# riddhiman13/predictive-multi-agent-framework

Measured on AMD Instinct MI355X. Metric: agent_rollouts_per_s, higher is better.
Workload: dtype f64; 1 GPU; C2: 64 agents x 200-step horizon, 32 sphere obstacles + repulsive sentinel, 1 population(s) per GPU (1 in the job) on 1 GPU(s), static obstacles, one pmaf_tick per step; agents=64, horizon=200, obstacles=32, populations_per_gpu=1, populations_total=1, parallelism=population-per-gpu x1 (same scene on every GPU), devices_visible=1, lanes_per_agent=64, rollout_blocks=64

## Files before the change

### include/pmaf.h

```cpp
#ifndef PMAF_H
#define PMAF_H

#include <stddef.h>
#include <stdint.h>

#ifdef __cplusplus
extern "C" {
#endif

#define PMAF_ABI_VERSION 7

typedef enum pmaf_status {
  PMAF_OK = 0,
  PMAF_ERR_INVALID = -1,
  PMAF_ERR_DEVICE = -2,
  PMAF_ERR_STATE = -3,
  PMAF_ERR_NOMEM = -4
} pmaf_status;

typedef enum pmaf_agent_type {
  PMAF_REAL_AGENT = 0,
  PMAF_GOAL_HEURISTIC = 1,
  PMAF_OBSTACLE_HEURISTIC = 2,
  PMAF_GOAL_OBSTACLE_HEURISTIC = 3,
// ... 141 lines not shown
int pmaf_set_profiling(pmaf_planner *h, int32_t enable);
int pmaf_get_launch_count(pmaf_planner *h, int64_t *launches);
int pmaf_get_kernel_stats(pmaf_planner *h, double *rollout_ms, int64_t *launches,
                          int64_t *agent_steps);
int pmaf_reset_kernel_stats(pmaf_planner *h);
int pmaf_get_launch_config(pmaf_planner *h, int32_t *lanes_per_agent,
                           int32_t *n_blocks, int32_t *lds_bytes);
int pmaf_get_waves_per_agent(pmaf_planner *h, int32_t *waves_per_agent, int32_t *obstacles_per_wave);
int pmaf_get_priority_slices(pmaf_planner *h, int32_t *enabled, int32_t *slice_ticks, int32_t *younger_of_8);
int32_t pmaf_pick_lanes_per_agent(int32_t n_agents, int32_t n_populations, int32_t n_field_obstacles, int32_t n_simds);
double pmaf_estimate_rollout_us(int32_t lanes_per_agent, int32_t n_agents, int32_t n_populations, int32_t n_field_obstacles,
                                int32_t horizon, int32_t n_simds);

int pmaf_debug_external_rollout(pmaf_planner *h, const char *code_object_path, const char *kernel_name);
int pmaf_debug_withhold_mailbox(pmaf_planner *h, int32_t enable);

int pmaf_debug_math(int32_t op, int32_t n, const double *a, const double *b, double *out);

#ifdef __cplusplus
}
#endif
#endif
```

### predictive-multi-agent-framework_amd/csrc/pmaf_host.cpp

```cpp
#include <hip/hip_runtime_api.h>
#include <unistd.h>

#include <cmath>
#include <cstdio>
#include <cstdlib>
#include <cstring>
#include <string>
#include <algorithm>
#include <chrono>
#include <thread>
#include <vector>

#include "../../include/pmaf.h"
#include "pmaf_comm.hpp"
#include "pmaf_types.hpp"
#include "pmaf_lpa_model.hpp"

#ifndef PMAF_W64_SLICE_DEFAULT
#define PMAF_W64_SLICE_DEFAULT true
#endif

using namespace pmaf;

static thread_local std::string g_err;
// ... 39 lines not shown
  size_t lds_rollout = 0, lds_manager = 0;
  hipModule_t ext_mod = nullptr;
  hipFunction_t ext_fn = nullptr;
  hipStream_t stream = nullptr;
  hipEvent_t ev_mgr = nullptr;
  uint64_t mailbox_seq = 0;
  double tick_timeout_s = 5.0;
  bool dbg_withhold = false;
  double *h_wp = nullptr, *d_wp = nullptr, *h_wph = nullptr, *d_wph = nullptr;
  std::vector<int32_t> wp_np, wp_agent;
  double wp_seq = 0.0;
  std::chrono::steady_clock::time_point last_tick_entry{};
  bool wp_timed = true;
  std::vector<double> wp_us;
  bool closest_dirty = true;
  std::vector<double> last_live;
  std::vector<double> live_resident;
  void note_live_obstacles(const double *obstacles) {
    const size_t row = (size_t)D.n_obs * 7, field = (size_t)(D.n_obs - 1) * 7;
    bool same = last_live.size() == (size_t)D.P * field;
    for (int p = 0; p < D.P && same; p++)
      same = std::memcmp(last_live.data() + p * field, obstacles + p * row, sizeof(double) * field) == 0;
    if (same) return;
    last_live.resize((size_t)D.P * field);
    for (int p = 0; p < D.P; p++) std::memcpy(last_live.data() + p * field, obstacles + p * row, sizeof(double) * field);
    closest_dirty = true;
  }
  bool uses_closest_table() const {
    const int M = D.n_obs - 1;
    const int tiles64 = (M >= 61 && M <= 64) ? 2 : (M + 63) / 64;
    return lpa == 64 && tiles64 >= 2 && tiles64 <= 4 && !force_generic;
  }
  static constexpr size_t TICK_RING = 8192;
  std::vector<float> tick_enq_us, tick_sp_us;
  size_t tick_head = 0, tick_count = 0;
  std::vector<void *> allocs;
  std::vector<size_t> alloc_bytes;
  double *h_out = nullptr;
  std::vector<double> real_pos_h, real_vel_h, real_force_h;
  double *d_out = nullptr;
  double *h_zc = nullptr, *d_zc = nullptr;
// ... 261 lines not shown

static void ensure_scores(pmaf_planner *h) {
  if (h->scores_valid) return;
  pmaf_k_launch_score(h->D, h->cp, h->stream);
  HIP_CHECK(hipGetLastError());
  h->scores_valid = true;
}

static const double *stage_live_obstacles_zero_copy(pmaf_planner *h, const double *obstacles) {
  if (!obstacles) return nullptr;
  const size_t n = (size_t)h->D.P * h->D.n_obs * 7;
  if (!h->peer.on && h->live_resident.size() == n && std::memcmp(h->live_resident.data(), obstacles, sizeof(double) * n) == 0) return nullptr;
  check_range(obstacles, n, "obstacles");
  h->note_live_obstacles(obstacles);
  h->live_resident.assign(obstacles, obstacles + n);
  aos_to_soa(obstacles, h->h_zc, h->D.P, h->D.n_obs);
  return h->d_zc;
}

struct ResidentGuard {
  pmaf_planner *h; bool armed = true;
  ~ResidentGuard() { if (armed) { h->live_resident.clear(); h->last_live.clear(); h->closest_dirty = true; } }
};

static void flush_real_position(pmaf_planner *h) {
  if (!h->real_pos_pending) return;
  sync(h);
  h->upload(h->D.real_pos, h->real_pos_h.data(), (size_t)h->D.P * 3);
  h->real_pos_pending = false;
}

static void launch_manager(pmaf_planner *h, const ManagerArgs &A0, hipEvent_t done = nullptr) {
  ManagerArgs A = A0;
  const bool hand_over_position = h->real_pos_pending;
  if (hand_over_position) {
    if (h->D.P <= PMAF_RP_INLINE) {
      A.real_pos_inline = 1;
      std::memcpy(A.real_pos_val, h->h_rp, sizeof(double) * 3 * (size_t)h->D.P);
    } else {
      A.real_pos_src = h->d_rp;
    }
  }
  if (A.do_reset) h->paths_gen++;
  if (A.do_reset && h->uses_closest_table()) { A.compute_closest = h->closest_dirty ? 1 : 0; h->closest_dirty = false; }
  A.tuned_real_step = (h->math == MATH_XACT && !h->force_generic) ? 1 : 0;
  pmaf_k_launch_manager(h->D, h->cp, A, h->lds_manager, h->stream, done);
  HIP_CHECK(hipGetLastError());
  if (hand_over_position) h->real_pos_pending = false;
}

static void refresh_real_cache(pmaf_planner *h) {
  for (int p = 0; p < h->D.P; p++) {
    const double *o = h->h_out + p * PMAF_MBOX;
    for (int c = 0; c < 3; c++) {
      h->real_pos_h[p * 3 + c] = o[1 + c];
      h->real_vel_h[p * 3 + c] = o[4 + c];
      h->real_force_h[p * 3 + c] = o[8 + c];
    }
  }
}

static void wait_mailbox(pmaf_planner *h, double seq, const char *who = "pmaf_tick") {
// ... 316 lines not shown
    REQUIRE(h->lds_manager <= 160 * 1024,
            "pmaf_create: n_agents + obstacle table exceed the manager kernel's LDS budget (160 KB: 8 B per agent, 60 B per obstacle)");
    HIP_CHECK(pmaf_k_set_lds_limits(h->lds_manager, h->lds_rollout));

    size_t PN = (size_t)P * N;
    double *goal = h->dalloc<double>(P * 3);
    D.goal = goal;
    D.agent_init_pos = h->dalloc<double>(P * 3);
    D.start_pos = h->dalloc<double>(P * 3);
    D.start_vel = h->dalloc<double>(P * 3);
    D.obs_start = h->dalloc<double>((size_t)P * 7 * n_obs);
    D.known_start = h->dalloc<int32_t>((size_t)P * n_obs);
    D.obs_live = h->dalloc<double>((size_t)P * 7 * n_obs);
    D.closest_idx = h->dalloc<int32_t>((size_t)P * n_obs);
    D.closest_ok = h->dalloc<int32_t>((size_t)P);
    double *ka = h->dalloc<double>(PN), *kc = h->dalloc<double>(PN), *kr = h->dalloc<double>(PN), *kd = h->dalloc<double>(PN);
    D.k_attr = ka; D.k_circ = kc; D.k_repel = kr; D.k_damp = kd;
    int32_t *types = h->dalloc<int32_t>(N);
    D.types = types;
    D.rot = h->dalloc<double>(PN * 3 * n_obs);
    double *rnd = h->dalloc<double>(PN * 3 * n_obs);
    D.rnd = rnd;
    D.paths = h->dalloc<double>(PN * (size_t)cap * 3);
    D.n_points = h->dalloc<int32_t>(PN);
    D.agent_vel = h->dalloc<double>(PN * 3);
    D.min_obs = h->dalloc<double>(PN);
    D.cost_ws = h->dalloc<double>(PN);
    D.path_len = h->dalloc<double>(PN);
    D.goal_dist = h->dalloc<double>(PN);
    D.reached = h->dalloc<int32_t>(PN);
// ... 81 lines not shown
        int p = (int)(pa / N);
        for (int c = 0; c < 3; c++) paths[pa * cap * 3 + c] = init[p * 3 + c];
        av[pa * 3] = 0.01;
      }
      h->upload(D.paths, paths.data(), paths.size());
      h->upload(D.n_points, np.data(), np.size());
      h->upload(D.min_obs, mo.data(), mo.size());
      h->upload(D.agent_vel, av.data(), av.size());
    }
    h->real_pos_h = init;
    h->real_vel_h = v0;
    h->real_force_h.assign(P * 3, 0.0);
    h->real_path.assign(P, {});
    for (int p = 0; p < P; p++) h->real_path[p].insert(h->real_path[p].end(), {init[p * 3], init[p * 3 + 1], init[p * 3 + 2]});
    h->rollout_pending = true;
    sync(h);
    *out = h;
  });
  if (rc != PMAF_OK && h) { pmaf_destroy(h); }
  return rc;
}

int pmaf_destroy(pmaf_planner *h) {
  if (!h) return PMAF_OK;
  (void)hipSetDevice(h->device);
  if (h->stream) (void)hipStreamSynchronize(h->stream);
  detach_comm(h);
  peer_disconnect(h);
  if (h->d_send1) (void)hipFree(h->d_send1);
  if (h->ext_mod) (void)hipModuleUnload(h->ext_mod);
// ... 17 lines not shown
}

int pmaf_set_initial_position(pmaf_planner *h, const double *pos) {
  return guarded([&] {
    REQUIRE(h && pos, "pmaf_set_initial_position: NULL argument");
    check_range(pos, (size_t)h->D.P * 3, "pmaf_set_initial_position");
    h->use_device();
    sync(h);
    DevView &D = h->D;
    const int P = D.P;
    h->upload(D.agent_init_pos, pos, P * 3);
    h->upload(D.real_init_pos, pos, P * 3);
    h->upload(D.real_pos, pos, P * 3);
    h->real_pos_pending = false;
    h->upload(D.start_pos, pos, P * 3);
    h->paths_gen++;
    pmaf_k_launch_restart_paths(D, D.start_pos, h->stream);
    HIP_CHECK(hipGetLastError());
    h->real_pos_h.assign(pos, pos + P * 3);
    for (int p = 0; p < P; p++)
      h->real_path[p].insert(h->real_path[p].end(), {pos[p * 3], pos[p * 3 + 1], pos[p * 3 + 2]});
    sync(h);
    h->scores_valid = false;
    h->rollout_pending = true;
    h->stepped = false;
  });
}

int pmaf_set_real_position(pmaf_planner *h, const double *pos) {
  return guarded([&] {
// ... 288 lines not shown
  const int P = h->D.P;
  check_range(pos, (size_t)P * 3, "pos");
  if (vel) check_range(vel, (size_t)P * 3, "vel");
  h->use_device();
  sync(h);
  std::vector<double> in((size_t)P * 6, 0.0);
  for (int p = 0; p < P; p++)
    for (int c = 0; c < 3; c++) { in[p * 6 + c] = pos[p * 3 + c]; if (vel) in[p * 6 + 3 + c] = vel[p * 3 + c]; }
  std::vector<double> pk((size_t)P * 6);
  for (int p = 0; p < P; p++)
    for (int c = 0; c < 3; c++) { pk[p * 3 + c] = in[p * 6 + c]; pk[(size_t)P * 3 + p * 3 + c] = in[p * 6 + 3 + c]; }
  h->upload(h->d_reset_in, pk.data(), pk.size());
  h->paths_gen++;
  pmaf_k_launch_set_agents(h->D, h->d_reset_in, vel ? h->d_reset_in + (size_t)P * 3 : nullptr, h->stream);
  HIP_CHECK(hipGetLastError());
  sync(h);
  h->scores_valid = false;
  h->rollout_pending = false;
  h->stepped = true;
}

int pmaf_set_agent_positions(pmaf_planner *h, const double *pos) {
  return guarded([&] {
    REQUIRE(h && pos, "pmaf_set_agent_positions: NULL argument");
    set_agents(h, pos, nullptr);
  });
}

int pmaf_set_agent_pos_and_vels(pmaf_planner *h, const double *pos, const double *vel) {
  return guarded([&] {
// ... 549 lines not shown

int pmaf_get_health(pmaf_planner *h, int32_t *bits) {
  return guarded([&] {
    REQUIRE(h && bits, "pmaf_get_health: NULL argument");
    for (int p = 0; p < h->D.P; p++) bits[p] = (int32_t)h->h_out[p * PMAF_MBOX + 15];
  });
}

int pmaf_debug_withhold_mailbox(pmaf_planner *h, int32_t enable) {
  return guarded([&] {
    REQUIRE(h, "pmaf_debug_withhold_mailbox: NULL handle");
    h->dbg_withhold = enable != 0;
  });
}

int pmaf_enable_winner_path(pmaf_planner *h, int32_t enable) {
  return guarded([&] {
    REQUIRE(h, "pmaf_enable_winner_path: NULL handle");
    h->use_device();
    sync(h);
    if (!enable) {
      if (h->h_wp) { (void)hipHostFree(h->h_wp); h->h_wp = nullptr; h->d_wp = nullptr; }
      if (h->h_wph) { (void)hipHostFree(h->h_wph); h->h_wph = nullptr; h->d_wph = nullptr; }
      h->wp_seq = 0.0;
      return;
    }
    if (h->h_wp) return;
    const size_t P = (size_t)h->D.P;
    HIP_CHECK(hipHostMalloc((void **)&h->h_wp, sizeof(double) * P * h->D.cap * 3, hipHostMallocMapped));
    HIP_CHECK(hipHostGetDevicePointer((void **)&h->d_wp, h->h_wp, 0));
// ... 159 lines not shown
      uint64_t n = 0;
      REQUIRE(r + sizeof(n) <= end, "pmaf_load_state: blob truncated");
      std::memcpy(&n, r, sizeof(n)); r += sizeof(n);
      REQUIRE(r + sizeof(double) * n <= end, "pmaf_load_state: blob truncated");
      rp.assign(reinterpret_cast<const double *>(r), reinterpret_cast<const double *>(r) + n);
      r += sizeof(double) * n;
    }
    h->paths_gen++;
    h->cp_valid = hd.cp_valid != 0;
    h->scores_valid = hd.scores_valid != 0;
    h->rollout_pending = hd.rollout_pending != 0;
    h->stepped = hd.stepped != 0;
    h->real_pos_pending = false;
    h->has_best_h = -1;
    h->closest_dirty = true;
    h->last_live.clear();
    h->live_resident.clear();
  });
}

void *pmaf_stream(pmaf_planner *h) { return h ? (void *)h->stream : nullptr; }

int pmaf_set_profiling(pmaf_planner *h, int32_t enable) {
  return guarded([&] {
    REQUIRE(h, "pmaf_set_profiling: NULL handle");
    h->use_device();
    sync(h);
    h->profiling = enable != 0;
    h->prof_every = enable > 1 ? enable : 1;
    h->prof_phase = 0;
// ... 102 lines not shown
```

### predictive-multi-agent-framework_amd/csrc/pmaf_k_misc.hip

```cpp
#include <mutex>
#include <hip/hip_runtime.h>
#include <hip/hip_ext.h>

#include "pmaf_types.hpp"
#include "pmaf_device.hpp"
#include "pmaf_rollout_w64.hpp"
#include "pmaf_rollout_grp.hpp"

using namespace pmaf;

template <int LPA>
__global__ __launch_bounds__(64) void k_rollout(DevView D, CostParams CP) {
  extern __shared__ double smem[];
  const int lane = threadIdx.x;
  const int pop = blockIdx.y;
  constexpr int APW = 64 / LPA;
  const int sub = lane % LPA;
  const int grp = lane / LPA;
  const int a = blockIdx.x * APW + grp;
  const bool active = a < D.N;
  const int aa = active ? a : 0;
  const int n_obs = D.n_obs;
  const PopConst C = D.C;
  const unsigned long long t_begin = wall_clock64();
// ... 209 lines not shown
  int best = D.best_idx[pop];
  const int had_best = D.has_best[pop];
  const int old_best_id = D.best_id[pop];
  int htype = D.best_type[pop];
  const double *rp_src = A.real_pos_src ? A.real_pos_src : D.real_pos;
  V3 rp;
  if (A.real_pos_inline) rp = mk(A.real_pos_val[pop * 3], A.real_pos_val[pop * 3 + 1], A.real_pos_val[pop * 3 + 2]);
  else rp = mk(rp_src[pop * 3], rp_src[pop * 3 + 1], rp_src[pop * 3 + 2]);
  if ((A.real_pos_src || A.real_pos_inline) && !A.do_move && lane == 0) {
    D.real_pos[pop * 3] = rp.x; D.real_pos[pop * 3 + 1] = rp.y; D.real_pos[pop * 3 + 2] = rp.z;
  }
  V3 rv = mk(D.real_vel[pop * 3], D.real_vel[pop * 3 + 1], D.real_vel[pop * 3 + 2]);
  V3 rf = mk(D.real_force[pop * 3], D.real_force[pop * 3 + 1], D.real_force[pop * 3 + 2]);
  const V3 init_pos = mk(D.real_init_pos[pop * 3], D.real_init_pos[pop * 3 + 1], D.real_init_pos[pop * 3 + 2]);
  int32_t *rk = D.real_known + (size_t)pop * n_obs;
  double *live_dev = D.obs_live + (size_t)pop * 7 * n_obs;
  const double *live = A.live_src ? A.live_src + (size_t)pop * 7 * n_obs : live_dev;
  if (A.do_move || A.do_reset) {
    if (A.live_src) {
      const int total = 7 * n_obs;
      for (int base = 0; base < total; base += 64 * 8) {
        double v[8];
#pragma unroll
        for (int k = 0; k < 8; k++) {
          const int i = base + k * 64 + lane;
          v[k] = (i < total) ? __builtin_nontemporal_load(live + i) : 0.0;
        }
#pragma unroll
        for (int k = 0; k < 8; k++) {
          const int i = base + k * 64 + lane;
          if (i < total) { smem[i] = v[k]; live_dev[i] = v[k]; }
        }
      }
    } else {
      for (int i = lane; i < 7 * n_obs; i += 64) smem[i] = live[i];
    }
    for (int i = lane; i < n_obs; i += 64) s_known[i] = rk[i];
  }
  unsigned long long peer_wait = 0ull;
  int peer_status = 0;
  const PeerView *PV = A.peer;
  const bool peer_on = PV != nullptr && A.do_select && A.do_move && A.do_reset;
  if (peer_on) {
    const int src_rank = PV->couple[pop * 2], src_pop = PV->couple[pop * 2 + 1];
    if (src_rank >= 0) {
      const double want = A.peer_tick - 1.0;
      const double *slot = PV->inbox + ((((size_t)((long long)want & 1) * PV->world + src_rank) * PV->P + src_pop) * PMAF_PEER_SLOT);
      const unsigned long long t0 = wall_clock64();
      for (;;) {
        const double got = __hip_atomic_load(slot + 8, __ATOMIC_ACQUIRE, __HIP_MEMORY_SCOPE_SYSTEM);
        if (got == want) break;
        if (got > want) { peer_status = 2; break; }
// ... 75 lines not shown
      const double *src = D.rnd + ((size_t)pop * N + min_idx) * 3 * n_obs;
      double *dst = D.best_rnd + (size_t)pop * 3 * n_obs;
      for (int i = lane; i < 3 * n_obs; i += 64) dst[i] = src[i];
      rand_g = src;
      htype = D.types[min_idx];
      if (lane == 0) {
        D.has_best[pop] = 1;
        D.best_id[pop] = min_idx + 1;
        D.best_type[pop] = htype;
      }
    }
    best = min_idx;
    if (lane == 0) D.best_idx[pop] = best;
  }
  PMAF_MSEC();
  if (A.do_move) {
    int gid = A.agent_id_inline ? A.agent_id_val[pop] : (A.agent_id ? A.agent_id[pop] : best);
    size_t pg = (size_t)pop * N + gid;
    double k_attr = D.k_attr[pg], k_circ = D.k_circ[pg], k_repel = D.k_repel[pg], k_damp = D.k_damp[pg];
    wave_lds_fence();
    const int ntiles = (M + 63) / 64;
    unsigned long long kb = 0ull;
    V3 F = mk(0.0, 0.0, 0.0);
    bool acc_clamped = false;
    if (A.tuned_real_step && ntiles <= 4) {
      double *rrot = D.real_rot + (size_t)pop * 3 * n_obs;
      double *clist = s_cost + N + (N & 1);
      unsigned kb32 = 0u;
      if (ntiles <= 1)
        real_step_w64<1>(D, A.dt_real, pop, lane, htype, smem, s_known, rrot, rand_g, clist, k_attr, k_circ, k_repel,
// ... 15 lines not shown
      bool gate = !(dg < C.approach || (norm(rv) < 0.5 * C.vel_max && norm(rp - init_pos) < 0.2));
      double scale = 1.0, dummy_min = C.shell;
      circ_and_scale<64, true>(gate, lane, 0, htype, rp, rv, goal, g, C, k_circ, T, n_obs,
                               D.real_rot + (size_t)pop * 3 * n_obs, rand_g, kb, dummy_min, F, scale);
      V3 new_pos;
      finish_step(rp, rv, g, F, scale, C, k_attr, k_repel, k_damp, A.dt_real, T.pos(n_obs - 1), T.r[n_obs - 1], new_pos);
      rp = new_pos;
      acc_clamped = norm((C.mass != 1.0) ? (F / C.mass) : F) > 13.0;
    }
    if (acc_clamped) health |= PMAF_HB_ACC_CLAMPED;
    rf = F;
    for (int t = 0; t < ntiles; t++) {
      int i = t * 64 + lane;
      if (i < M) {
        const int32_t f = (int32_t)((kb >> t) & 1ull);
        rk[i] = f;
        s_known[i] = f;
      }
    }
    if (lane == 0) {
      D.real_pos[pop * 3] = rp.x; D.real_pos[pop * 3 + 1] = rp.y; D.real_pos[pop * 3 + 2] = rp.z;
      D.real_vel[pop * 3] = rv.x; D.real_vel[pop * 3 + 1] = rv.y; D.real_vel[pop * 3 + 2] = rv.z;
      D.real_force[pop * 3] = F.x; D.real_force[pop * 3 + 1] = F.y; D.real_force[pop * 3 + 2] = F.z;
    }
  }

  PMAF_MSEC();
  double hv[PMAF_WINNER_HDR];
  const bool want_hdr = A.do_select && (A.winner_hdr != nullptr || peer_on);
  if (want_hdr) {
    const size_t pb = (size_t)pop * N + best;
    hv[0] = s_cost[best];
    hv[1] = (double)best;
    hv[2] = (double)D.n_points[pb];
// ... 62 lines not shown
    double *wh = A.wp_hdr + pop * 4;
    if (lane == 0) { wh[0] = (double)(n3 / 3); wh[1] = (double)best; wh[2] = 0.0; }
    __threadfence_system();
    if (lane == 0) *reinterpret_cast<volatile double *>(wh + 3) = A.seq;
  }
  if (A.do_reset) {
    V3 sp, sv;
    if (A.reset_from_real) { sp = rp; sv = rv; }
    else if (A.reset_in_inline) {
      sp = mk(A.reset_in_val[pop * 6], A.reset_in_val[pop * 6 + 1], A.reset_in_val[pop * 6 + 2]);
      sv = mk(A.reset_in_val[pop * 6 + 3], A.reset_in_val[pop * 6 + 4], A.reset_in_val[pop * 6 + 5]);
    } else { sp = reset_sp; sv = reset_sv; }
    double vn = norm(sv);
    if (vn > C.vel_max) sv = (C.vel_max / vn) * sv;
    wave_lds_fence();
    double *st = D.obs_start + (size_t)pop * 7 * n_obs;
    for (int i = lane; i < 6 * n_obs; i += 64) st[i] = smem[i];
    int32_t *ks = D.known_start + (size_t)pop * n_obs;
    for (int i = lane; i < n_obs; i += 64) ks[i] = s_known[i];
    if (!A.rollout_follows) {
      for (int a = lane; a < N; a += 64) {
        size_t pa = (size_t)pop * N + a;
        double *path = D.paths + pa * (size_t)D.cap * 3;
        path[0] = sp.x; path[1] = sp.y; path[2] = sp.z;
        D.n_points[pa] = 1;
        D.agent_vel[pa * 3] = sv.x; D.agent_vel[pa * 3 + 1] = sv.y; D.agent_vel[pa * 3 + 2] = sv.z;
        D.min_obs[pa] = C.shell;
      }
      int32_t *ko = D.known_out + (size_t)pop * N * n_obs;
      for (int k = lane; k < N * n_obs; k += 64) ko[k] = s_known[k % n_obs];
    }
    if (lane == 0) {
      D.start_pos[pop * 3] = sp.x; D.start_pos[pop * 3 + 1] = sp.y; D.start_pos[pop * 3 + 2] = sp.z;
      D.start_vel[pop * 3] = sv.x; D.start_vel[pop * 3 + 1] = sv.y; D.start_vel[pop * 3 + 2] = sv.z;
    }
    if (A.compute_closest) {
      bool mv = false;
      for (int i = lane; i < M; i += 64) {
        const V3 ov = T.vel(i);
        mv = mv || !(ov.x == 0.0 && ov.y == 0.0 && ov.z == 0.0);
      }
      mv = wave_any(mv);
      if (!mv) {
        int32_t *ci = D.closest_idx + (size_t)pop * n_obs;
        for (int i = lane; i < M; i += 64) ci[i] = closest_other(T, n_obs, i, T.pos(i));
      }
      if (lane == 0) D.closest_ok[pop] = mv ? 0 : 1;
    }
  }
// ... 180 lines not shown
  const int pop = idx / D.N;
  const V3 q = mk(pos[pop * 3], pos[pop * 3 + 1], pos[pop * 3 + 2]);
  double *path = D.paths + (size_t)idx * D.cap * 3;
  path[0] = q.x; path[1] = q.y; path[2] = q.z;
  D.n_points[idx] = 1;
  V3 w = mk(0.0, 0.0, 0.0);
  if (vel) {
    w = mk(vel[pop * 3], vel[pop * 3 + 1], vel[pop * 3 + 2]);
    const double vn = norm(w);
    if (vn > D.C.vel_max) w = (D.C.vel_max / vn) * w;
    D.agent_vel[idx * 3] = w.x; D.agent_vel[idx * 3 + 1] = w.y; D.agent_vel[idx * 3 + 2] = w.z;
  }
  if (idx % D.N == 0) {
    D.start_pos[pop * 3] = q.x; D.start_pos[pop * 3 + 1] = q.y; D.start_pos[pop * 3 + 2] = q.z;
    if (vel) { D.start_vel[pop * 3] = w.x; D.start_vel[pop * 3 + 1] = w.y; D.start_vel[pop * 3 + 2] = w.z; }
  }
}

__global__ void k_eval_obstacle_distance(DevView D, const double *obs, double *out) {
  const int idx = blockIdx.x * blockDim.x + threadIdx.x;
  if (idx >= D.P * D.N) return;
  const int pop = idx / D.N;
  const int n_obs = D.n_obs;
  const double *o = obs + (size_t)pop * 7 * n_obs;
  const double *path = D.paths + (size_t)idx * D.cap * 3;
  const int n = D.n_points[idx];
  const V3 p = mk(path[(n - 1) * 3], path[(n - 1) * 3 + 1], path[(n - 1) * 3 + 2]);
  double min_dist = D.C.shell;
  for (int k = 0; k < n_obs; k++) {
    const double d = norm(p - mk(o[k], o[n_obs + k], o[2 * n_obs + k])) - (D.C.rad + o[6 * n_obs + k]);
// ... 126 lines not shown
```

### predictive-multi-agent-framework_amd/csrc/pmaf_k_w64.hip

```cpp
#include <hip/hip_runtime.h>
#include <hip/hip_ext.h>

#include "pmaf_types.hpp"
#include "pmaf_device.hpp"
#include "pmaf_rollout_w64.hpp"
#include "pmaf_rollout_grp.hpp"

using namespace pmaf;

__device__ __forceinline__ double *w64_exp_lds() {
  __shared__ double s_expk[EXPK_N];
  return s_expk;
}
template <int TILES>
__device__ __forceinline__ auto w64_exp_consts(int lane) {
  if constexpr (TILES >= 2) {
    double *tab = w64_exp_lds();
    exp_consts_to_lds(tab, lane);
    wave_lds_fence();
    return exp_consts_from_lds(tab);
  } else {
    return exp_consts_in_vgprs();
  }
}
// ... 252 lines not shown
    D.cost_ws[pa] = cost_ws;
    D.path_len[pa] = path_len;
    D.goal_dist[pa] = dg;
    if (ran) D.reached[pa] = dg < 0.100001;
    atomicAdd(D.step_counter, (unsigned long long)(n - 1));
    D.pred_ticks[pa] = wall_clock64() - t_begin;
  }
}

template <int TILES, int MATH, bool DPPSUM, bool PLAIN, bool SLICE>
__device__ __forceinline__ void rollout_w64_dispatch(const DevView &D, const CostParams &CP) {
  const int lane = threadIdx.x;
  const int pop = blockIdx.y;
  const int a = blockIdx.x;
  if (TILES == 1) {
    const int n_obs = D.n_obs, M = n_obs - 1;
    const double *src = D.obs_start + (size_t)pop * 7 * n_obs;
    const V3 sp = mk(src[M], src[n_obs + M], src[2 * n_obs + M]);
    const V3 sv = mk(src[3 * n_obs + M], src[4 * n_obs + M], src[5 * n_obs + M]);
    const V3 p0 = mk(D.start_pos[pop * 3], D.start_pos[pop * 3 + 1], D.start_pos[pop * 3 + 2]);
    const PopConst C0 = D.C;
    const bool reach = sentinel_reachable(p0, sp, sv, D.zsent_lt[pop], C0, D.cap);
    bool rest = true;
    for (int i = lane; i < M; i += 64) {
      const unsigned long long bx = (unsigned long long)__double_as_longlong(src[3 * n_obs + i]),
                               by = (unsigned long long)__double_as_longlong(src[4 * n_obs + i]),
                               bz = (unsigned long long)__double_as_longlong(src[5 * n_obs + i]);
      rest = rest && ((bx | by | bz) == 0ull);
    }
    const bool st = !wave_any(!rest) && (M <= 59 || !reach);
#define PMAF_BODY(T) \
    if (st) { \
      if (!reach) rollout_w64_body<TILES, T, MATH, 0, DPPSUM, PLAIN, true, SLICE>(D, CP, lane, pop, a); \
      else rollout_w64_body<TILES, T, MATH, 1, DPPSUM, PLAIN, true, SLICE>(D, CP, lane, pop, a); \
    } else if (!reach) rollout_w64_body<TILES, T, MATH, 0, DPPSUM, PLAIN, false, SLICE>(D, CP, lane, pop, a); \
    else rollout_w64_body<TILES, T, MATH, 1, DPPSUM, PLAIN, false, SLICE>(D, CP, lane, pop, a)
    switch (D.types[a]) {
      case T_GOAL: PMAF_BODY(T_GOAL); break;
      case T_OBST: PMAF_BODY(T_OBST); break;
      case T_GOALOBST: PMAF_BODY(T_GOALOBST); break;
      case T_VEL: PMAF_BODY(T_VEL); break;
      case T_RANDOM: PMAF_BODY(T_RANDOM); break;
      case T_HAD: PMAF_BODY(T_HAD); break;
      default: break;
    }
#undef PMAF_BODY
    return;
  }
  switch (D.types[a]) {
    case T_GOAL: rollout_w64_body<TILES, T_GOAL, MATH, 2, DPPSUM, PLAIN>(D, CP, lane, pop, a); break;
    case T_OBST: rollout_w64_body<TILES, T_OBST, MATH, 2, DPPSUM, PLAIN>(D, CP, lane, pop, a); break;
    case T_GOALOBST: rollout_w64_body<TILES, T_GOALOBST, MATH, 2, DPPSUM, PLAIN>(D, CP, lane, pop, a); break;
// ... 55 lines not shown
```

### predictive-multi-agent-framework_amd/csrc/pmaf_types.hpp

```cpp
#pragma once
#include <hip/hip_runtime_api.h>
#include <stddef.h>
#include <stdint.h>

#define PMAF_WINNER_HDR 8
#define PMAF_MBOX 16
#define PMAF_HB_SETPOINT_NAN 1
#define PMAF_HB_FORCE_NAN 2
#define PMAF_HB_ACC_CLAMPED 4
#define PMAF_HB_COST_NAN 8
#define PMAF_PEER_SLOT 16
#define PMAF_PEER_MAX_WORLD 64

namespace pmaf {

enum : int { MATH_IEEE = 0, MATH_FAST = 1, MATH_XACT = 2, MATH_FMA = 3 };

constexpr int pmaf_list_area_doubles(int slots_per_lane) { return (64 * (slots_per_lane <= 2 ? 2 : 4) + 8 + 64) * 4; }

struct PopConst {
  double dt, vel_max, approach, shell, mass, rad;
  double zf_gt, zacc_gt, zinit_lt, zvhalf_lt, zv09_lt;
};

// ... 25 lines not shown
  double *costs;
  double *real_pos, *real_vel, *real_force, *real_init_pos;
  int32_t *real_known;
  double *real_rot;
  int32_t *has_best, *best_id, *best_type;
  double *best_rnd;
  int32_t *best_idx;
  unsigned long long *step_counter;
  unsigned long long *pred_ticks;
  const double *zsent_lt;
  int ablate;
  int n_simds;
  int prio_slice_log2, prio_younger_of_8;
  int32_t *closest_idx;
  int32_t *closest_ok;
};

struct CostParams {
  double k_goal_dist, k_path_len, k_safe_dist, k_workspace;
  double ws[6];
};


struct PeerView {
  int world, rank, P, pad;
  double *inbox;
  double *peer[PMAF_PEER_MAX_WORLD];
  const int32_t *couple;
  const double *couple_radius;
  unsigned long long timeout_ticks;
// ... 2 lines not shown
struct ManagerArgs {
  int do_select, do_move, do_reset;
  int reset_from_real;
  int rollout_follows;
  int tuned_real_step;
  const double *live_src;
  double dt_real;
  const int32_t *agent_id;
  const double *reset_in;
  double *out;
  double seq;
  const PeerView *peer;
  double peer_tick;
  double *winner_hdr;
  int winner_stride;
  int compute_closest;
  double *wp_out;
  double *wp_hdr;
  const double *real_pos_src;
  int real_pos_inline;
  double real_pos_val[3 * 4];
  int agent_id_inline;
  int32_t agent_id_val[4];
  int reset_in_inline;
  double reset_in_val[6 * 4];
};
#define PMAF_RP_INLINE 4

struct PlanArgs {
  const double *obs;
// ... 30 lines not shown
```

### predictive-multi-agent-framework_amd/planner.py

```python
import ctypes as C
import os

import numpy as np

_HERE = os.path.dirname(os.path.abspath(__file__))
VARIANT = os.environ.get("PMAF_VARIANT", "")
LIB_PATH = os.environ.get("PMAF_LIB_PATH") or os.path.join(_HERE, "lib_" + VARIANT if VARIANT else "lib", "libpmaf_hip.so")

_dp = C.POINTER(C.c_double)
_ip = C.POINTER(C.c_int32)


class PmafError(RuntimeError):
    def __init__(self, code, msg):
        super().__init__("pmaf status %d: %s" % (code, msg))
        self.code = code


class PmafParams(C.Structure):
    _fields_ = [
        ("abi_version", C.c_int32), ("n_populations", C.c_int32), ("n_agents", C.c_int32),
        ("n_obstacles", C.c_int32), ("max_prediction_steps", C.c_int32), ("device", C.c_int32),
        ("lanes_per_agent", C.c_int32), ("flags", C.c_int32),
        ("dt", C.c_double), ("velocity_max", C.c_double), ("approach_dist", C.c_double),
# ... 72 lines not shown
    "pmaf_get_kernel_stats": (C.c_int, [_V, _dp, C.POINTER(C.c_int64), C.POINTER(C.c_int64)]),
    "pmaf_reset_kernel_stats": (C.c_int, [_V]),
    "pmaf_get_launch_count": (C.c_int, [_V, C.POINTER(C.c_int64)]),
    "pmaf_get_launch_config": (C.c_int, [_V, _ip, _ip, _ip]),
    "pmaf_get_waves_per_agent": (C.c_int, [_V, _ip, _ip]),
    "pmaf_get_priority_slices": (C.c_int, [_V, _ip, _ip, _ip]),
    "pmaf_pick_lanes_per_agent": (C.c_int32, [C.c_int32, C.c_int32, C.c_int32, C.c_int32]),
    "pmaf_estimate_rollout_us": (C.c_double, [C.c_int32, C.c_int32, C.c_int32, C.c_int32, C.c_int32, C.c_int32]),
    "pmaf_debug_math": (C.c_int, [C.c_int32, C.c_int32, _dp, _dp, _dp]),
    "pmaf_debug_external_rollout": (C.c_int, [_V, C.c_char_p, C.c_char_p]),
    "pmaf_get_health": (C.c_int, [_V, _ip]),
    "pmaf_enable_winner_path": (C.c_int, [_V, C.c_int32]),
    "pmaf_view_winner_path": (C.c_int, [_V, C.POINTER(_dp), C.POINTER(_ip), C.POINTER(_ip)]),
    "pmaf_get_winner_path_times_us": (C.c_int, [_V, _dp, C.c_int32, _ip]),
    "pmaf_debug_withhold_mailbox": (C.c_int, [_V, C.c_int32]),
    "pmaf_peer_info": (C.c_int, [_V, _ip, _ip]),
}


def debug_math(op, a, b=None):
    L = load_library()
    a = np.ascontiguousarray(a, dtype=np.float64)
    b = np.ascontiguousarray(a if b is None else b, dtype=np.float64)
    out = np.zeros_like(a)
    rc = L.pmaf_debug_math(op, a.size, a.ctypes.data_as(_dp), b.ctypes.data_as(_dp), out.ctypes.data_as(_dp))
    if rc != 0:
        raise PmafError(rc, L.pmaf_last_error().decode())
    return out

_LIB = None
# ... 316 lines not shown
        paths = [full[p, :n[p]].copy() for p in range(self.P)]
        return (paths[0], int(n[0]), int(a[0])) if self.P == 1 else (paths, n, a)

    def winner_path_wait(self):
        self._chk(self.L.pmaf_view_winner_path(self._h, None, None, None))

    def winner_path_times_us(self, max_n=1 << 16):
        out = np.zeros(max_n)
        n = C.c_int32(0)
        self._chk(self.L.pmaf_get_winner_path_times_us(self._h, _p(out), max_n, C.byref(n)))
        return out[:n.value].copy()

    def debug_withhold_mailbox(self, enable=True):
        self._chk(self.L.pmaf_debug_withhold_mailbox(self._h, 1 if enable else 0))

    def peer_info(self):
        f, w = C.c_int32(0), C.c_int32(0)
        self._chk(self.L.pmaf_peer_info(self._h, C.byref(f), C.byref(w)))
        return {"fine_grained": bool(f.value), "world": w.value}

    PEER_HANDLE_BYTES = 128

    def peer_export(self, world):
        buf = (C.c_ubyte * self.PEER_HANDLE_BYTES)()
        self._chk(self.L.pmaf_peer_export(self._h, int(world), C.cast(buf, C.c_void_p)))
        return bytes(buf)

    def peer_connect(self, world, rank, handles):
        blob = b"".join(handles)
        assert len(blob) == world * self.PEER_HANDLE_BYTES
# ... 171 lines not shown
```

Before: 270,000 rollouts/s.

## Precompute rollout dispatch facts in manager and skip redundant start-state copies

The manager kernel now computes, once per reset, whether all obstacles are at rest and whether the sentinel is reachable, and stores both in a small device array. Each rollout block reads these flags instead of rescanning the obstacle velocities and re-running the reachability test. The manager also skips rewriting obs_start and known_start when host-side flags show they are already in sync, and it batches the LDS fill of the obstacle and known arrays. In exchange it adds invalidation bookkeeping across reset, set-position and peer paths, with a risk of using stale flags if any invalidation is missed.

```diff
diff --git a/include/pmaf.h b/include/pmaf.h
--- a/include/pmaf.h
+++ b/include/pmaf.h
@@ -179,6 +179,7 @@
 
 int pmaf_debug_external_rollout(pmaf_planner *h, const char *code_object_path, const char *kernel_name);
 int pmaf_debug_withhold_mailbox(pmaf_planner *h, int32_t enable);
+int pmaf_debug_dispatch_facts(pmaf_planner *h, int32_t *facts);
 
 int pmaf_debug_math(int32_t op, int32_t n, const double *a, const double *b, double *out);
 
diff --git a/predictive-multi-agent-framework_amd/csrc/pmaf_host.cpp b/predictive-multi-agent-framework_amd/csrc/pmaf_host.cpp
--- a/predictive-multi-agent-framework_amd/csrc/pmaf_host.cpp
+++ b/predictive-multi-agent-framework_amd/csrc/pmaf_host.cpp
@@ -77,6 +77,9 @@
   bool wp_timed = true;
   std::vector<double> wp_us;
   bool closest_dirty = true;
+  bool facts_off = false;
+  bool rest_dirty = true;
+  bool obs_synced = false, known_synced = false;
   std::vector<double> last_live;
   std::vector<double> live_resident;
   void note_live_obstacles(const double *obstacles) {
@@ -88,6 +91,13 @@
     last_live.resize((size_t)D.P * field);
     for (int p = 0; p < D.P; p++) std::memcpy(last_live.data() + p * field, obstacles + p * row, sizeof(double) * field);
     closest_dirty = true;
+    rest_dirty = true;
+  }
+  void invalidate_facts() {
+    HIP_CHECK(hipMemsetAsync(D.disp_facts, 0xFF, sizeof(int32_t) * 2 * (size_t)D.P, stream));
+    rest_dirty = true;
+    obs_synced = false;
+    known_synced = false;
   }
   bool uses_closest_table() const {
     const int M = D.n_obs - 1;
@@ -379,13 +389,19 @@
   check_range(obstacles, n, "obstacles");
   h->note_live_obstacles(obstacles);
   h->live_resident.assign(obstacles, obstacles + n);
+  h->obs_synced = false;
   aos_to_soa(obstacles, h->h_zc, h->D.P, h->D.n_obs);
   return h->d_zc;
 }
 
 struct ResidentGuard {
   pmaf_planner *h; bool armed = true;
-  ~ResidentGuard() { if (armed) { h->live_resident.clear(); h->last_live.clear(); h->closest_dirty = true; } }
+  ~ResidentGuard() {
+    if (armed) {
+      h->live_resident.clear(); h->last_live.clear(); h->closest_dirty = true;
+      h->rest_dirty = true; h->obs_synced = false; h->known_synced = false;
+    }
+  }
 };
 
 static void flush_real_position(pmaf_planner *h) {
@@ -409,8 +425,21 @@
   if (A.do_reset) h->paths_gen++;
   if (A.do_reset && h->uses_closest_table()) { A.compute_closest = h->closest_dirty ? 1 : 0; h->closest_dirty = false; }
   A.tuned_real_step = (h->math == MATH_XACT && !h->force_generic) ? 1 : 0;
+  if (A.do_reset) {
+    A.facts_off = h->facts_off ? 1 : 0;
+    A.compute_rest = h->rest_dirty ? 1 : 0;
+    A.obs_unchanged = (!h->facts_off && h->obs_synced && !h->peer.on) ? 1 : 0;
+    A.start_synced = (!h->facts_off && h->known_synced) ? 1 : 0;
+  }
   pmaf_k_launch_manager(h->D, h->cp, A, h->lds_manager, h->stream, done);
   HIP_CHECK(hipGetLastError());
+  if (A.do_reset) {
+    h->rest_dirty = false;
+    h->obs_synced = !h->peer.on;
+    h->known_synced = true;
+  } else if (A.do_move) {
+    h->known_synced = false;
+  }
   if (hand_over_position) h->real_pos_pending = false;
 }
 
@@ -757,6 +786,7 @@
     D.obs_live = h->dalloc<double>((size_t)P * 7 * n_obs);
     D.closest_idx = h->dalloc<int32_t>((size_t)P * n_obs);
     D.closest_ok = h->dalloc<int32_t>((size_t)P);
+    D.disp_facts = h->dalloc<int32_t>((size_t)P * 2);
     double *ka = h->dalloc<double>(PN), *kc = h->dalloc<double>(PN), *kr = h->dalloc<double>(PN), *kd = h->dalloc<double>(PN);
     D.k_attr = ka; D.k_circ = kc; D.k_repel = kr; D.k_damp = kd;
     int32_t *types = h->dalloc<int32_t>(N);
@@ -868,6 +898,8 @@
     h->real_path.assign(P, {});
     for (int p = 0; p < P; p++) h->real_path[p].insert(h->real_path[p].end(), {init[p * 3], init[p * 3 + 1], init[p * 3 + 2]});
     h->rollout_pending = true;
+    { const char *e = getenv("PMAF_DISPATCH_FACTS"); h->facts_off = e && e[0] == '0'; }
+    h->invalidate_facts();
     sync(h);
     *out = h;
   });
@@ -915,6 +947,7 @@
     h->upload(D.real_pos, pos, P * 3);
     h->real_pos_pending = false;
     h->upload(D.start_pos, pos, P * 3);
+    h->invalidate_facts();
     h->paths_gen++;
     pmaf_k_launch_restart_paths(D, D.start_pos, h->stream);
     HIP_CHECK(hipGetLastError());
@@ -1233,6 +1266,7 @@
   h->paths_gen++;
   pmaf_k_launch_set_agents(h->D, h->d_reset_in, vel ? h->d_reset_in + (size_t)P * 3 : nullptr, h->stream);
   HIP_CHECK(hipGetLastError());
+  h->rest_dirty = true; h->obs_synced = false; h->known_synced = false;
   sync(h);
   h->scores_valid = false;
   h->rollout_pending = false;
@@ -1812,6 +1846,15 @@
   });
 }
 
+int pmaf_debug_dispatch_facts(pmaf_planner *h, int32_t *facts) {
+  return guarded([&] {
+    REQUIRE(h && facts, "pmaf_debug_dispatch_facts: NULL argument");
+    h->use_device();
+    sync(h);
+    h->download(facts, h->D.disp_facts, (size_t)h->D.P * 2);
+  });
+}
+
 int pmaf_enable_winner_path(pmaf_planner *h, int32_t enable) {
   return guarded([&] {
     REQUIRE(h, "pmaf_enable_winner_path: NULL handle");
@@ -2001,6 +2044,7 @@
     h->real_pos_pending = false;
     h->has_best_h = -1;
     h->closest_dirty = true;
+    h->invalidate_facts();
     h->last_live.clear();
     h->live_resident.clear();
   });
diff --git a/predictive-multi-agent-framework_amd/csrc/pmaf_k_misc.hip b/predictive-multi-agent-framework_amd/csrc/pmaf_k_misc.hip
--- a/predictive-multi-agent-framework_amd/csrc/pmaf_k_misc.hip
+++ b/predictive-multi-agent-framework_amd/csrc/pmaf_k_misc.hip
@@ -247,6 +247,10 @@
   V3 rf = mk(D.real_force[pop * 3], D.real_force[pop * 3 + 1], D.real_force[pop * 3 + 2]);
   const V3 init_pos = mk(D.real_init_pos[pop * 3], D.real_init_pos[pop * 3 + 1], D.real_init_pos[pop * 3 + 2]);
   int32_t *rk = D.real_known + (size_t)pop * n_obs;
+  int32_t *facts = D.disp_facts + (size_t)pop * 2;
+  int rest_fact = -1;
+  double zsent_lt = 0.0;
+  if (A.do_reset) { rest_fact = facts[0]; zsent_lt = D.zsent_lt[pop]; }
   double *live_dev = D.obs_live + (size_t)pop * 7 * n_obs;
   const double *live = A.live_src ? A.live_src + (size_t)pop * 7 * n_obs : live_dev;
   if (A.do_move || A.do_reset) {
@@ -265,10 +269,35 @@
           if (i < total) { smem[i] = v[k]; live_dev[i] = v[k]; }
         }
       }
+      for (int i = lane; i < n_obs; i += 64) s_known[i] = rk[i];
     } else {
-      for (int i = lane; i < 7 * n_obs; i += 64) smem[i] = live[i];
-    }
-    for (int i = lane; i < n_obs; i += 64) s_known[i] = rk[i];
+      const int total = 7 * n_obs;
+      int32_t kf[8];
+#pragma unroll
+      for (int k = 0; k < 8; k++) {
+        const int i = k * 64 + lane;
+        kf[k] = (i < n_obs) ? rk[i] : 0;
+      }
+      for (int base = 0; base < total; base += 64 * 8) {
+        double v[8];
+#pragma unroll
+        for (int k = 0; k < 8; k++) {
+          const int i = base + k * 64 + lane;
+          v[k] = (i < total) ? live[i] : 0.0;
+        }
+#pragma unroll
+        for (int k = 0; k < 8; k++) {
+          const int i = base + k * 64 + lane;
+          if (i < total) smem[i] = v[k];
+        }
+      }
+#pragma unroll
+      for (int k = 0; k < 8; k++) {
+        const int i = k * 64 + lane;
+        if (i < n_obs) s_known[i] = kf[k];
+      }
+      for (int i = 512 + lane; i < n_obs; i += 64) s_known[i] = rk[i];
+    }
   }
   unsigned long long peer_wait = 0ull;
   int peer_status = 0;
@@ -374,6 +403,7 @@
     if (lane == 0) D.best_idx[pop] = best;
   }
   PMAF_MSEC();
+  bool latched = false;
   if (A.do_move) {
     int gid = A.agent_id_inline ? A.agent_id_val[pop] : (A.agent_id ? A.agent_id[pop] : best);
     size_t pg = (size_t)pop * N + gid;
@@ -419,10 +449,12 @@
       int i = t * 64 + lane;
       if (i < M) {
         const int32_t f = (int32_t)((kb >> t) & 1ull);
+        latched = latched || (f != s_known[i]);
         rk[i] = f;
         s_known[i] = f;
       }
     }
+    latched = wave_any(latched);
     if (lane == 0) {
       D.real_pos[pop * 3] = rp.x; D.real_pos[pop * 3 + 1] = rp.y; D.real_pos[pop * 3 + 2] = rp.z;
       D.real_vel[pop * 3] = rv.x; D.real_vel[pop * 3 + 1] = rv.y; D.real_vel[pop * 3 + 2] = rv.z;
@@ -515,10 +547,23 @@
     double vn = norm(sv);
     if (vn > C.vel_max) sv = (C.vel_max / vn) * sv;
     wave_lds_fence();
+    if (A.compute_rest) {
+      bool nz = false;
+      for (int i = lane; i < M; i += 64) {
+        const unsigned long long bx = (unsigned long long)__double_as_longlong(smem[3 * n_obs + i]),
+                                 by = (unsigned long long)__double_as_longlong(smem[4 * n_obs + i]),
+                                 bz = (unsigned long long)__double_as_longlong(smem[5 * n_obs + i]);
+        nz = nz || ((bx | by | bz) != 0ull);
+      }
+      rest_fact = wave_any(nz) ? 0 : 1;
+    }
+    if (A.facts_off) rest_fact = -1;
     double *st = D.obs_start + (size_t)pop * 7 * n_obs;
-    for (int i = lane; i < 6 * n_obs; i += 64) st[i] = smem[i];
+    if (!(A.obs_unchanged && rest_fact == 1))
+      for (int i = lane; i < 6 * n_obs; i += 64) st[i] = smem[i];
     int32_t *ks = D.known_start + (size_t)pop * n_obs;
-    for (int i = lane; i < n_obs; i += 64) ks[i] = s_known[i];
+    if (!(A.start_synced && !latched))
+      for (int i = lane; i < n_obs; i += 64) ks[i] = s_known[i];
     if (!A.rollout_follows) {
       for (int a = lane; a < N; a += 64) {
         size_t pa = (size_t)pop * N + a;
@@ -534,6 +579,10 @@
     if (lane == 0) {
       D.start_pos[pop * 3] = sp.x; D.start_pos[pop * 3 + 1] = sp.y; D.start_pos[pop * 3 + 2] = sp.z;
       D.start_vel[pop * 3] = sv.x; D.start_vel[pop * 3 + 1] = sv.y; D.start_vel[pop * 3 + 2] = sv.z;
+      int reach_fact = sentinel_reachable(sp, T.pos(M), T.vel(M), zsent_lt, C, D.cap) ? 1 : 0;
+      if (A.facts_off) reach_fact = -1;
+      if (A.compute_rest || A.facts_off) facts[0] = rest_fact;
+      facts[1] = reach_fact;
     }
     if (A.compute_closest) {
       bool mv = false;
@@ -744,6 +793,7 @@
   if (idx % D.N == 0) {
     D.start_pos[pop * 3] = q.x; D.start_pos[pop * 3 + 1] = q.y; D.start_pos[pop * 3 + 2] = q.z;
     if (vel) { D.start_vel[pop * 3] = w.x; D.start_vel[pop * 3 + 1] = w.y; D.start_vel[pop * 3 + 2] = w.z; }
+    D.disp_facts[pop * 2] = -1; D.disp_facts[pop * 2 + 1] = -1;
   }
 }
 
diff --git a/predictive-multi-agent-framework_amd/csrc/pmaf_k_w64.hip b/predictive-multi-agent-framework_amd/csrc/pmaf_k_w64.hip
--- a/predictive-multi-agent-framework_amd/csrc/pmaf_k_w64.hip
+++ b/predictive-multi-agent-framework_amd/csrc/pmaf_k_w64.hip
@@ -290,28 +290,38 @@
   const int pop = blockIdx.y;
   const int a = blockIdx.x;
   if (TILES == 1) {
-    const int n_obs = D.n_obs, M = n_obs - 1;
-    const double *src = D.obs_start + (size_t)pop * 7 * n_obs;
-    const V3 sp = mk(src[M], src[n_obs + M], src[2 * n_obs + M]);
-    const V3 sv = mk(src[3 * n_obs + M], src[4 * n_obs + M], src[5 * n_obs + M]);
-    const V3 p0 = mk(D.start_pos[pop * 3], D.start_pos[pop * 3 + 1], D.start_pos[pop * 3 + 2]);
-    const PopConst C0 = D.C;
-    const bool reach = sentinel_reachable(p0, sp, sv, D.zsent_lt[pop], C0, D.cap);
-    bool rest = true;
-    for (int i = lane; i < M; i += 64) {
-      const unsigned long long bx = (unsigned long long)__double_as_longlong(src[3 * n_obs + i]),
-                               by = (unsigned long long)__double_as_longlong(src[4 * n_obs + i]),
-                               bz = (unsigned long long)__double_as_longlong(src[5 * n_obs + i]);
-      rest = rest && ((bx | by | bz) == 0ull);
-    }
-    const bool st = !wave_any(!rest) && (M <= 59 || !reach);
+    const int32_t *facts = D.disp_facts + (size_t)pop * 2;
+    const int f_rest = facts[0], f_reach = facts[1];
+    const int type = D.types[a];
+    bool reach, rest_all;
+    if (f_rest >= 0 && f_reach >= 0) {
+      reach = f_reach != 0;
+      rest_all = f_rest != 0;
+    } else {
+      const int n_obs = D.n_obs, M = n_obs - 1;
+      const double *src = D.obs_start + (size_t)pop * 7 * n_obs;
+      const V3 sp = mk(src[M], src[n_obs + M], src[2 * n_obs + M]);
+      const V3 sv = mk(src[3 * n_obs + M], src[4 * n_obs + M], src[5 * n_obs + M]);
+      const V3 p0 = mk(D.start_pos[pop * 3], D.start_pos[pop * 3 + 1], D.start_pos[pop * 3 + 2]);
+      const PopConst C0 = D.C;
+      reach = sentinel_reachable(p0, sp, sv, D.zsent_lt[pop], C0, D.cap);
+      bool rest = true;
+      for (int i = lane; i < M; i += 64) {
+        const unsigned long long bx = (unsigned long long)__double_as_longlong(src[3 * n_obs + i]),
+                                 by = (unsigned long long)__double_as_longlong(src[4 * n_obs + i]),
+                                 bz = (unsigned long long)__double_as_longlong(src[5 * n_obs + i]);
+        rest = rest && ((bx | by | bz) == 0ull);
+      }
+      rest_all = !wave_any(!rest);
+    }
+    const bool st = rest_all && (D.n_obs - 1 <= 59 || !reach);
 #define PMAF_BODY(T) \
     if (st) { \
       if (!reach) rollout_w64_body<TILES, T, MATH, 0, DPPSUM, PLAIN, true, SLICE>(D, CP, lane, pop, a); \
       else rollout_w64_body<TILES, T, MATH, 1, DPPSUM, PLAIN, true, SLICE>(D, CP, lane, pop, a); \
     } else if (!reach) rollout_w64_body<TILES, T, MATH, 0, DPPSUM, PLAIN, false, SLICE>(D, CP, lane, pop, a); \
     else rollout_w64_body<TILES, T, MATH, 1, DPPSUM, PLAIN, false, SLICE>(D, CP, lane, pop, a)
-    switch (D.types[a]) {
+    switch (type) {
       case T_GOAL: PMAF_BODY(T_GOAL); break;
       case T_OBST: PMAF_BODY(T_OBST); break;
       case T_GOALOBST: PMAF_BODY(T_GOALOBST); break;
diff --git a/predictive-multi-agent-framework_amd/csrc/pmaf_types.hpp b/predictive-multi-agent-framework_amd/csrc/pmaf_types.hpp
--- a/predictive-multi-agent-framework_amd/csrc/pmaf_types.hpp
+++ b/predictive-multi-agent-framework_amd/csrc/pmaf_types.hpp
@@ -63,6 +63,7 @@
   int prio_slice_log2, prio_younger_of_8;
   int32_t *closest_idx;
   int32_t *closest_ok;
+  int32_t *disp_facts;
 };
 
 struct CostParams {
@@ -95,6 +96,7 @@
   double peer_tick;
   double *winner_hdr;
   int winner_stride;
+  int compute_rest, facts_off, obs_unchanged, start_synced;
   int compute_closest;
   double *wp_out;
   double *wp_hdr;
diff --git a/predictive-multi-agent-framework_amd/planner.py b/predictive-multi-agent-framework_amd/planner.py
--- a/predictive-multi-agent-framework_amd/planner.py
+++ b/predictive-multi-agent-framework_amd/planner.py
@@ -110,6 +110,7 @@
     "pmaf_view_winner_path": (C.c_int, [_V, C.POINTER(_dp), C.POINTER(_ip), C.POINTER(_ip)]),
     "pmaf_get_winner_path_times_us": (C.c_int, [_V, _dp, C.c_int32, _ip]),
     "pmaf_debug_withhold_mailbox": (C.c_int, [_V, C.c_int32]),
+    "pmaf_debug_dispatch_facts": (C.c_int, [_V, _ip]),
     "pmaf_peer_info": (C.c_int, [_V, _ip, _ip]),
 }
 
@@ -456,6 +457,11 @@
     def debug_withhold_mailbox(self, enable=True):
         self._chk(self.L.pmaf_debug_withhold_mailbox(self._h, 1 if enable else 0))
 
+    def debug_dispatch_facts(self):
+        out = np.zeros((self.P, 2), dtype=np.int32)
+        self._chk(self.L.pmaf_debug_dispatch_facts(self._h, out.ctypes.data_as(_ip)))
+        return out
+
     def peer_info(self):
         f, w = C.c_int32(0), C.c_int32(0)
         self._chk(self.L.pmaf_peer_info(self._h, C.byref(f), C.byref(w)))
```

New measurement: 269,400 rollouts/s. About the same (-0.2%).
